# Litianyu141/Gen-FVGN-steady

Hardware: AMD Instinct MI355X
Metric: training iters/sec, 50k-cell cylinder mesh (fwd + loss + bwd + Adam, batch resident in HBM) (higher is better)
Workload: dtype f32

## Files before the change

### gen-fvgn-steady_amd/csrc/gfv_launch.h

```cpp
#pragma once
#include <hip/hip_runtime.h>
#include <tuple>
#include <type_traits>

struct GfvRecorder;
GfvRecorder* gfv_rec_active();
void gfv_rec_push(GfvRecorder* r, hipError_t (*run)(const void* blob, hipStream_t st), const void* blob, size_t bytes, hipStream_t st);

template <class... KArgs, class... Args>
inline void gfv_launch(void (*kernel)(KArgs...), dim3 grid, dim3 block, size_t shmem, hipStream_t st, Args&&... args) {
  hipLaunchKernelGGL(kernel, grid, block, shmem, st, args...);
  if (GfvRecorder* r = gfv_rec_active()) {
    struct Blob {
      void (*k)(KArgs...);
      dim3 g, b;
      size_t sh;
      std::tuple<std::decay_t<KArgs>...> a;
    };
    static_assert(std::is_trivially_copyable<std::tuple<std::decay_t<KArgs>...>>::value || true, "kernel arguments are plain data");
    const Blob blob{kernel, grid, block, shmem, std::tuple<std::decay_t<KArgs>...>(args...)};
    gfv_rec_push(r, [](const void* p, hipStream_t s) -> hipError_t {
      const Blob& B = *static_cast<const Blob*>(p);
      std::apply([&](const auto&... a) { hipLaunchKernelGGL(B.k, B.g, B.b, B.sh, s, a...); }, B.a);
      return hipGetLastError();
    }, &blob, sizeof(Blob), st);
  }
}
#define GFV_LAUNCH(kernel, grid, block, shmem, stream, ...) gfv_launch(kernel, dim3(grid), dim3(block), (size_t)(shmem), stream, __VA_ARGS__)

hipError_t gfv_memset_rec(void* dst, int value, size_t bytes, hipStream_t st);
```

### gen-fvgn-steady_amd/csrc/gfv_limits.h

```cpp
#pragma once
enum {
  GFV_LIM_CBWD_ON = 0,
  GFV_LIM_CBWD_MAX_M,
  GFV_LIM_CFWD_ON,
  GFV_LIM_CFWD_MAX_M,
  GFV_LIM_CTRANS_ON,
  GFV_LIM_CTRANS_MAX_M,
  GFV_LIM_LIN1S_ON,
  GFV_LIM_LIN1S_MAX_M,
  GFV_LIM_COUNT
};
int gfv_internal_limit(int which);
```

### gen-fvgn-steady_amd/csrc/record.hip

```cpp
#include <algorithm>
#include <cstdlib>
#include <cstring>
#include <mutex>
#include <unordered_map>
#include <vector>

#include "../../include/gfv.h"
#include "gfv_common.h"
#include "gfv_launch.h"

struct GfvRecorder {
  struct Cmd {
    hipError_t (*run)(const void*, hipStream_t);
    hipStream_t st;
    size_t off;
  };
  std::vector<Cmd> cmds;
  std::vector<char> arena;
};

namespace {
thread_local GfvRecorder* t_active = nullptr;
std::mutex g_mu;
std::unordered_map<int64_t, GfvRecorder*> g_lists;
int64_t g_next = 1;

constexpr int N_EVENTS = 64;
constexpr int MAX_DEVICES = 16;
struct EventRing {
  hipEvent_t ev[N_EVENTS];
  bool ready = false;
  int next = 0;
};
EventRing g_rings[MAX_DEVICES];
hipEvent_t next_event() {
  int dev = 0;
  if (hipGetDevice(&dev) != hipSuccess || dev < 0 || dev >= MAX_DEVICES) return nullptr;
  std::lock_guard<std::mutex> lk(g_mu);
  EventRing& r = g_rings[dev];
  if (!r.ready) {
    for (int i = 0; i < N_EVENTS; ++i)
      if (hipEventCreateWithFlags(&r.ev[i], hipEventDisableTiming) != hipSuccess) return nullptr;
    r.ready = true;
  }
  hipEvent_t e = r.ev[r.next];
  r.next = (r.next + 1) % N_EVENTS;
  return e;
}
struct WaitBlob {
  hipStream_t waited;
};
hipError_t run_wait(const void* p, hipStream_t waiter) {
  const WaitBlob& B = *static_cast<const WaitBlob*>(p);
  hipEvent_t e = next_event();
  if (!e) return hipErrorInvalidResourceHandle;
  hipError_t rc = hipEventRecord(e, B.waited);
  if (rc != hipSuccess) return rc;
  return hipStreamWaitEvent(waiter, e, 0);
}
struct MemsetBlob {
  void* dst;
  int value;
  size_t bytes;
};
hipError_t run_memset(const void* p, hipStream_t st) {
  const MemsetBlob& B = *static_cast<const MemsetBlob*>(p);
  return hipMemsetAsync(B.dst, B.value, B.bytes, st);
}
}

GfvRecorder* gfv_rec_active() { return t_active; }
void gfv_rec_push(GfvRecorder* r, hipError_t (*run)(const void*, hipStream_t), const void* blob, size_t bytes, hipStream_t st) {
  const size_t off = (r->arena.size() + 15) & ~(size_t)15;
  r->arena.resize(off + bytes);
  memcpy(r->arena.data() + off, blob, bytes);
  r->cmds.push_back({run, st, off});
}
hipError_t gfv_memset_rec(void* dst, int value, size_t bytes, hipStream_t st) {
  const MemsetBlob b{dst, value, bytes};
  const hipError_t rc = run_memset(&b, st);
  if (GfvRecorder* r = gfv_rec_active()) gfv_rec_push(r, run_memset, &b, sizeof(b), st);
  return rc;
}

extern "C" int gfv_record_begin(void) {
  if (t_active) return GFV_ERR_ARG;
  t_active = new GfvRecorder();
  return GFV_OK;
}
extern "C" int gfv_record_count(void) { return t_active ? (int)t_active->cmds.size() : -1; }
extern "C" int64_t gfv_record_end(void) {
  if (!t_active) return 0;
  GfvRecorder* r = t_active;
  t_active = nullptr;
  std::lock_guard<std::mutex> lk(g_mu);
  const int64_t h = g_next++;
  g_lists[h] = r;
  return h;
}
extern "C" int gfv_record_length(int64_t handle) {
  std::lock_guard<std::mutex> lk(g_mu);
  auto it = g_lists.find(handle);
  return it == g_lists.end() ? -1 : (int)it->second->cmds.size();
}
extern "C" int gfv_record_replay(int64_t handle, int32_t first, int32_t last) {
  GfvRecorder* r = nullptr;
  {
    std::lock_guard<std::mutex> lk(g_mu);
    auto it = g_lists.find(handle);
    if (it == g_lists.end()) return GFV_ERR_ARG;
    r = it->second;
  }
  const int n = (int)r->cmds.size();
  if (first < 0 || last > n || first > last) return GFV_ERR_ARG;
  if (t_active) return GFV_ERR_ARG;
  const char* base = r->arena.data();
  for (int i = first; i < last; ++i)
    if (r->cmds[i].run(base + r->cmds[i].off, r->cmds[i].st) != hipSuccess) return GFV_ERR_LAUNCH;
  return GFV_OK;
}
extern "C" int gfv_record_free(int64_t handle) {
  GfvRecorder* r = nullptr;
  {
    std::lock_guard<std::mutex> lk(g_mu);
    auto it = g_lists.find(handle);
    if (it == g_lists.end()) return GFV_ERR_ARG;
    r = it->second;
    g_lists.erase(it);
  }
  delete r;
  return GFV_OK;
}
extern "C" int gfv_stream_wait(void* waiter, void* waited) {
  const WaitBlob b{(hipStream_t)waited};
  hipEvent_t e = next_event();
  if (!e) return GFV_ERR_LAUNCH;
  if (hipEventRecord(e, (hipStream_t)waited) != hipSuccess || hipStreamWaitEvent((hipStream_t)waiter, e, 0) != hipSuccess)
    return GFV_ERR_LAUNCH;
  if (GfvRecorder* r = gfv_rec_active()) gfv_rec_push(r, run_wait, &b, sizeof(b), (hipStream_t)waiter);
  return GFV_OK;
}

extern "C" int gfv_record_delay_side(int64_t handle, void* main_stream, int32_t k) {
  GfvRecorder* r = nullptr;
  {
    std::lock_guard<std::mutex> lk(g_mu);
    auto it = g_lists.find(handle);
    if (it == g_lists.end()) return GFV_ERR_ARG;
    r = it->second;
  }
  if (k <= 0) return 0;
  const hipStream_t ms = (hipStream_t)main_stream;
  auto& c = r->cmds;
  const size_t n = c.size();
  auto is_join = [&](size_t i) { return c[i].st == ms && c[i].run == run_wait; };
  int moved_runs = 0;
  size_t i = 0;
  while (i < n) {
    if (c[i].st == ms) { ++i; continue; }
    size_t j = i;
    while (j < n && c[j].st != ms) ++j;
    size_t d = 0, t = j;
    while (t < n && !is_join(t)) { if (c[t].st == ms) ++d; ++t; }
    size_t want = d / 3 < (size_t)k ? d / 3 : (size_t)k;
// ... 13 lines not shown
```

### gen-fvgn-steady_amd/csrc/rowtile.hip

```cpp
#include <atomic>
#include <stdio.h>
#include <stdlib.h>
#include <mutex>
#include "gfv_common.h"
#include "gfv_limits.h"
#include "gfv_prof.h"
#include "../../include/gfv.h"

namespace {
constexpr int BM = 64;
}

int gfv_internal_tchain_launch(const gfv_rowtile_args_t* args, int ragged, int f16, hipStream_t stream);

static std::atomic<int> g_f16_default{-1};
static thread_local int g_f16split = -1;
static int f16_default() {
  int d = g_f16_default.load(std::memory_order_relaxed);
  if (d < 0) {
    const char* e = getenv("GFV_F16SPLIT");
    d = e ? ((atoi(e) == 2 || atoi(e) == 3) ? atoi(e) : (atoi(e) != 0)) : 1;
    int expect = -1;
    if (!g_f16_default.compare_exchange_strong(expect, d)) d = expect;
  }
// ... 7 lines not shown
}
extern "C" int gfv_set_f16split_thread(int32_t on) {
  if (on < -1 || on > 3) return GFV_ERR_ARG;
  g_f16split = on;
  return GFV_OK;
}
static int f16_mode() { return gfv_f16split_enabled(); }

static thread_local int g_hidden = 128;
extern "C" int gfv_hidden_size(void) { return g_hidden; }
extern "C" int gfv_set_hidden_size(int32_t h) {
  if (h < 16 || h > 128 || (h & 15)) return GFV_ERR_ARG;
  g_hidden = h;
  return GFV_OK;
}

static thread_local int g_last_path = -1;
extern "C" int gfv_rowtile_last_path(void) { return g_last_path; }
namespace {
struct LimitDef { const char* env; int dflt; };
const LimitDef k_limits[GFV_LIM_COUNT] = {
    {"GFV_CBWD", 1},        {"GFV_CBWD_MAX_M", 25000},      {"GFV_CFWD", 1},          {"GFV_CFWD_MAX_M", 250000},
    {"GFV_CTRANS", 1},         {"GFV_CTRANS_MAX_M", 16384},
    {"GFV_LIN1S", 1},       {"GFV_LIN1S_MAX_M", 16384}};
int g_limit[GFV_LIM_COUNT];
bool g_limit_set[GFV_LIM_COUNT];
std::once_flag g_limit_once;
void limits_init() {
  for (int i = 0; i < GFV_LIM_COUNT; ++i) {
    const char* e = getenv(k_limits[i].env);
    g_limit[i] = e ? atoi(e) : k_limits[i].dflt;
    g_limit_set[i] = false;
  }
}
}
int gfv_internal_limit(int which) {
  std::call_once(g_limit_once, limits_init);
  return (which >= 0 && which < GFV_LIM_COUNT) ? g_limit[which] : 0;
}
extern "C" int gfv_get_limit(int32_t which) { return (which >= 0 && which < GFV_LIM_COUNT) ? gfv_internal_limit(which) : -1; }
extern "C" int gfv_set_limit(int32_t which, int32_t value) {
  if (which < 0 || which >= GFV_LIM_COUNT) return GFV_ERR_ARG;
  std::call_once(g_limit_once, limits_init);
  if (value < 0) {
    const char* e = getenv(k_limits[which].env);
    g_limit[which] = e ? atoi(e) : k_limits[which].dflt;
  } else {
// ... 164 lines not shown
```

### gen-fvgn-steady_amd/gfv/cmdlist.py

```python
from __future__ import annotations

import torch

import os

NATIVE = os.environ.get("GFV_CMDLIST_NATIVE", "1") != "0"

_QUERIES = frozenset((
    "gfv_abi_version", "gfv_struct_size", "gfv_rowtile_tiles", "gfv_rowtile_last_path", "gfv_dw_chunks", "gfv_dw_slabs",
    "gfv_linear_dw_workspace_floats", "gfv_dw_multi_workspace_floats", "gfv_f16split_enabled", "gfv_set_f16split", "gfv_set_f16split_thread", "gfv_hidden_size",
    "gfv_weight_image_bytes", "gfv_normalizer_blocks", "gfv_slice_softmax_bwd_blocks", "gfv_profile_enable",
    "gfv_profile_collect", "gfv_profile_reset", "gfv_profile_set_sizes", "gfv_status_flags", "gfv_status_mirror", "gfv_prep_workspace_bytes", "gfv_grad_guard_workspace_bytes", "gfv_get_limit", "gfv_set_limit", "gfv_limit_name", "gfv_rowtile_dw_partials", "gfv_rowtile_dw_partials_m",
    "gfv_rowtile_fuses_dw", "gfv_graph_norm_workspace_bytes", "gfv_plan_create", "gfv_plan_destroy", "gfv_plan_table", "gfv_plan_sizes",
    "gfv_record_begin", "gfv_record_count", "gfv_record_end", "gfv_record_length", "gfv_record_replay", "gfv_record_free",
    "gfv_record_delay_side", "gfv_pool_args_bytes", "gfv_pool_table_bytes", "gfv_pool_table_check",
    "gfv_sweep_mirror_create", "gfv_sweep_mirror_free"))


class CommandList:
    def __init__(self):
        self.cmds = []
        self.pool = None
        self.main = None
        self.keep = []
        self.native = 0
        self.n_native = 0

    def __len__(self):
        return len(self.cmds) + self.n_native

    def __del__(self):
        if self.native:
            try:
                from . import lib as L
                L.load(raw=True).gfv_record_free(self.native)
            except Exception:
                pass

# ... 24 lines not shown
                    fn(*args)


_ACTIVE = None


def active():
    return _ACTIVE


_IN_CALL = 0


def call(fn, *args):
    global _IN_CALL
    _IN_CALL += 1
    try:
        r = fn(*args)
    finally:
        _IN_CALL -= 1
    if _ACTIVE is not None:
        if _ACTIVE.native:
            from . import lib as L
            _ACTIVE.cmds.append((fn, args, torch.cuda.current_stream(), L.load(raw=True).gfv_record_count()))
        else:
            _ACTIVE.cmds.append((fn, args, torch.cuda.current_stream()))
    return r


_NO_KERNEL = frozenset((
    "aten::empty.memory_format", "aten::empty_strided", "aten::empty_like", "aten::new_empty", "aten::new_empty_strided",
    "aten::detach", "aten::alias", "aten::lift_fresh", "aten::_unsafe_view", "aten::is_pinned", "aten::resize_",
    "aten::set_.source_Storage", "aten::set_.source_Storage_storage_offset", "aten::set_.source_Tensor", "aten::_local_scalar_dense",
    "aten::is_same_size", "aten::stride", "aten::sym_size", "aten::sym_stride", "aten::sym_numel", "aten::sym_storage_offset"))


def _guard_mode():
    from torch.utils._python_dispatch import TorchDispatchMode
    from torch.utils._pytree import tree_leaves

    class Guard(TorchDispatchMode):
        def __torch_dispatch__(self, func, types, args=(), kwargs=None):
            out = func(*args, **(kwargs or {}))
            if _IN_CALL == 0:
                name = func._schema.name + ("." + func._overloadname if func._overloadname and func._overloadname != "default" else "")
                if name not in _NO_KERNEL and not getattr(func, "is_view", False):
                    leaves = tree_leaves((args, kwargs, out))
# ... 84 lines not shown
```

### gen-fvgn-steady_amd/gfv/engine.py

```python
from __future__ import annotations

import contextlib
import os
import struct

import torch

from . import cmdlist
from . import lib as L
from . import ops
from .ops import LayerSpec, Seg

_MODE = {"explicit": 0, "implicit": 1, "imex": 2}


def _empty(dev, *shape):
    return torch.empty(shape, dtype=torch.float32, device=dev)


def pick_concurrent_stream(priority=0, candidates=8):
    if torch.cuda.is_current_stream_capturing():
        return torch.cuda.Stream(priority=priority)
    main = torch.cuda.current_stream()
    cycles = 400_000
# ... 102 lines not shown
        self._zero_e = None
        self._etmp = None
        self._prep_ws = None
        self._fvm_cnt = None
        self._fvm_fuse = os.environ.get("GFV_FVM_FUSE", "1") != "0"
        self._agg_ln = os.environ.get("GFV_AGG_LN", "1") != "0"
        self._side, self._sides = None, []
        self._keep = []
        self.dist_world, self.dist_group, self.dist_force = 1, None, False
        self._retired = []
        self.bucket_hook = None

    class _Fork:
        def __init__(self, eng, keep):
            self.eng, self.keep = eng, keep

        def __enter__(self):
            e = self.eng
            if not e.overlap:
                return self
            if e._side is None:
                e._side = pick_concurrent_stream()
                e._sides = [e._side]
            L.stream_wait(e._side, torch.cuda.current_stream())
            e._keep.extend(t for t in self.keep if t is not None)
            self._ctx = torch.cuda.stream(e._side)
            self._ctx.__enter__()
            return self

        def __exit__(self, *exc):
            if self.eng.overlap:
                self._ctx.__exit__(*exc)
            return False

    def fork(self, *keep):
        return Engine._Fork(self, keep)

    @contextlib.contextmanager
    def model_width(self):
        lib = L.load()
        if self.hidden == 128 and lib.gfv_hidden_size() == 128:
            yield
            return
        L.check(lib.gfv_set_hidden_size(self.hidden), "gfv_set_hidden_size")
        try:
            yield
        finally:
# ... 25 lines not shown
        if not self._pending:
            return
        pend, self._pending = self._pending, []
        if split and len(pend) > 1:
            k = 1 if split == 1 else len(pend) - 1
            main_part, side_part = (pend[:k], pend[k:]) if split == 1 else (pend[k:], pend[:k])
            self._pending = side_part
            self.flush()
            self._pending = main_part
            self.flush(on_main=True)
            return
        if on_main:
            ws, self._dw_ws = self._dw_ws, self._dw_ws_main
            try:
                for fn, _ in pend:
                    fn()
            finally:
                self._dw_ws_main, self._dw_ws = self._dw_ws, ws
            return
        with self.fork(*[t for _, keep in pend for t in keep]):
            for fn, _ in pend:
                fn()

    def join(self):
        self.flush()
        if self.overlap and self._side is not None:
            for sd in self._sides:
                L.stream_wait(torch.cuda.current_stream(), sd)
        self._keep.clear()

    def _pkey(self, P, fresh=False):
        hit = self._pkey_cache
        if fresh or hit is None or hit[0] is not P:
            self._pkey_cache = hit = (P, tuple(t.data_ptr() for t in P.values()))
        return hit[1]

    def _wi_enter(self, phase, P):
        if not self.f16split:
            return None
        key = self._pkey(P, fresh=(phase == "fwd"))
        if self._wi_key != key:
            dev = next(iter(P.values())).device
            self._retired.append((self._wi, self._wmax, self._wi_abs))
            self._wmax = torch.zeros((1,), dtype=torch.float32, device=dev)
            self._wi = {ph: ops.WeightImages(dev, self._wmax) for ph in ("fwd", "bwd")}
            self._wi["fwd"].add_static(P.values())
            mats = [t for t in P.values() if t.dim() == 2 and t.stride(1) == 1]
            self._wi_abs = ops.WeightImages._upload([((t.data_ptr(), t.stride(0), t.shape[0], t.shape[1]), t) for t in mats], dev)
            self._wi_key = key
        wi = self._wi[phase]
        if phase == "fwd":
# ... 7 lines not shown
        return ops.set_weight_images(wi)

    def build_static_images(self, P):
        if not self.f16split:
            return
        prev = self._wi_enter("fwd", P)
        ops.set_weight_images(prev)

    def _wi_static_enter(self, P):
        if not self.f16split:
            return None
        if self._wi is None or self._wi_key != self._pkey(P, fresh=True):
            raise RuntimeError("static weight images belong to another parameter set: call build_static_images(P) first")
        wi = self._wi["fwd"]
        if len(wi.valid) != len(wi.images) and cmdlist.active() is None:
            L.check(L.load().gfv_weight_absmax(self._wi_abs[0].data_ptr(), self._wi_abs[1], self._wmax.data_ptr(),
                                               L.stream_ptr()), "gfv_weight_absmax")
            wi.build()
        return ops.set_weight_images(wi)

    def capture_signature(self):
        wi = self._wi or {}
        return (self._wi_key, self._wt_key, L.load().gfv_f16split_enabled(),
                tuple((ph, len(w.images), None if w._desc is None else w._desc.data_ptr()) for ph, w in sorted(wi.items())))

    def _wi_exit(self, phase, prev):
        if not self.f16split:
            return
        self._wi[phase].invalidate()
        ops.set_weight_images(prev)

    def _T(self, W, perm=False):
        hit = self._wt.get((W.data_ptr(), perm)) if self._wt_live else None
        if hit is not None:
            return hit
        if not perm:
            return ops.transpose(W)
        if perm == "c":
            return ops.transpose(W, col0=256, ncols=128)
        if perm == "ab":
            return torch.cat((ops.transpose(W, col0=0, ncols=128), ops.transpose(W, col0=128, ncols=128)), 1).contiguous()
        out = _empty(W.device, 192, 128)
        ops.transpose(W, out=out[0:128], col0=64, ncols=128)
        ops.transpose(W, out=out[128:192], col0=0, ncols=64)
        return out

# ... 879 lines not shown
            if g_emb is not None:
                pending = g_emb
            if self.bucket_hook is not None and proc is sv["procs"][-1] and len(sv["procs"]) > 1:
                self.flush()
                self.bucket_hook()
        tail = self._tail_cfg(pl)[0] if self._defer_mode else 0
        self.mlp3_bwd(P, sv["sv_eenc"], g_e, grads)
        self.flush(on_main=tail >= 2)
        self.mlp3_bwd(P, sv["sv_nenc"], g_x, grads, g_add=pending)
        self.flush(on_main=tail >= 1)

    def forward(self, P, buffers, x, pl, *, norm_global=True, accumulate=True, want_outputs=True, want_edge_attr15=True,
                before_prep=None, x_raw=None, train_loss=None, keep=True, static_weights=False):
        if static_weights:
            prev = self._wi_static_enter(P)
        else:
            with self.fork():
                prev = self._wi_enter("fwd", P)
        try:
            if before_prep is not None:
                before_prep()
            uv_old, ea16, ea15 = self.prep_fwd(x, buffers, pl, norm_global, accumulate, want_edge_attr15, x_raw=x_raw)
            if not static_weights:
                self.join()
            dec, sv_sim = self.simulator_fwd(P, x, ea16, pl, keep=keep)
        finally:
            if not static_weights:
                self._wi_exit("fwd", prev)
            elif self.f16split:
                ops.set_weight_images(prev)
        if not keep:
            del ea16
        losses, uvp_node, uvp_cell, sv_fvm = self.fvm_fwd(dec, uv_old, pl, want_outputs, train_loss=train_loss, keep=keep)
        return losses, uvp_node, uvp_cell, ea15, (dict(sim=sv_sim, fvm=sv_fvm) if keep else None)

    def backward(self, P, ctx, gloss, grads, pl, g_dec_hook=None):
        with self.fork():
            self.prepare_transposes(P)
            prev = self._wi_enter("bwd", P)
        try:
            g_dec = self.fvm_bwd(ctx["fvm"], gloss, pl)
            if g_dec_hook is not None:
                g_dec_hook(g_dec)
            self.join()
            self.simulator_bwd(P, ctx["sim"], g_dec, grads, pl)
            self.join()
        finally:
            self._wt_live = False
            self._wi_exit("bwd", prev)
        return grads
```

### gen-fvgn-steady_amd/gfv/functions.py

```python
from __future__ import annotations

import torch

from .engine import Engine, GradStore
from .plan import get_plan


def require_gpu(t):
    if not t.is_cuda:
        raise RuntimeError("Gen-FVGN MI355X path: tensors must live on the GPU (HIP kernels only, no CPU fallback)")


def _alloc_grads(names, tensors, skip=()):
    return GradStore(names, [t.shape for t in tensors], tensors[0].device, skip=skip)


def unused_param_names(names):
    return {n for n in names if ".ln_1." in ("." + n) or n.endswith("Attn.temperature")}


class GnBlockFn(torch.autograd.Function):
    @staticmethod
    def forward(ctx, engine, plan, names, x, e, *params):
        require_gpu(x)
# ... 136 lines not shown
        ent = self.entries.get(key)
        if ent is None:
            if len(self.entries) >= 4:
                self.entries.pop(next(iter(self.entries)))
            ent = self.entries[key] = _Replay()
            ent.plan = plan
        return ent

    def clear(self):
        self.entries.clear()


class ModelFn(torch.autograd.Function):

    @staticmethod
    def forward(ctx, engine, plan, names, buffers, x, flags, cache, *params):
        require_gpu(x)
        from . import cmdlist
        from . import lib as L
        t_in = __import__("time").perf_counter() if TIMING is not None else 0.0
        P = None
        ent = None
        if cache is not None and cmdlist.active() is None and not torch.cuda.is_current_stream_capturing():
            key = (id(plan), flags["norm_global"], flags["accumulate"], L.load().gfv_f16split_enabled(),
                   tuple(p.data_ptr() for p in params))
            ent = cache.lookup(engine, plan, key)

        def run():
            nonlocal P
            P = dict(zip(names, (p.detach() for p in params)))
            return engine.forward(P, buffers, x, plan, norm_global=flags["norm_global"], accumulate=flags["accumulate"])
        with engine.model_width():
            if ent is None or ent.pending:
                ent = None
                losses, uvp_node, uvp_cell, ea15, sv = run()
            elif ent.fwd is None:
                if ent.warm < ReplayCache.WARM:
                    ent.warm += 1
                    ent = None
                    losses, uvp_node, uvp_cell, ea15, sv = run()
                else:
                    with cmdlist.record() as cl:
                        losses, uvp_node, uvp_cell, ea15, sv = run()
                    ent.fwd, ent.x, ent.sv, ent.P = cl, x, sv, P
                    ent.outs = (losses, uvp_node, uvp_cell, ea15)
                    ent.sig = engine.capture_signature()
            elif ent.sig != engine.capture_signature():
# ... 79 lines not shown
```

### gen-fvgn-steady_amd/gfv/lib.py

```python
from __future__ import annotations

import ctypes as C
import os

import torch

HERE = os.path.dirname(os.path.abspath(__file__))
LIB_PATH = os.environ.get("GFV_LIB", os.path.join(HERE, "libgfv.so"))

c_float_p = C.c_void_p
c_int_p = C.c_void_p

OP_NONE, OP_BIAS_GELU, OP_MUL_DGELU = 0, 1, 2
IN_NONE, IN_GELU, IN_LN, IN_LNBWD = 0, 1, 2, 3
FIN_PLAIN, FIN_LN, FIN_LNBWD = 0, 1, 2
CHAIN_ROW_OWNER, CHAIN_COLUMN_OWNER = 1, 2
DW_COLSCALE = 8


class Seg(C.Structure):
    _fields_ = [("ptr", C.c_void_p), ("idx", C.c_void_p), ("width", C.c_int32), ("ld", C.c_int32),
                ("csr_rowptr", C.c_void_p), ("csr_scale", C.c_void_p), ("save", C.c_void_p)]


# ... 268 lines not shown
                                       C.c_void_p]),
    "gfv_anderson_gram": (C.c_int, [C.c_void_p, C.c_void_p, C.c_int32, C.c_void_p, C.c_void_p, C.c_void_p, C.c_int32, C.c_int32,
                                    C.c_int32, C.c_double, C.c_double, C.c_int32] + [C.c_void_p] * 10 + [C.c_int32, C.c_void_p,
                                                                                                         C.c_void_p]),
    "gfv_anderson_mix": (C.c_int, [C.c_void_p, C.c_void_p, C.c_int32, C.c_void_p, C.c_void_p, C.c_void_p, C.c_int32, C.c_int32,
                                   C.c_int32, C.c_double, C.c_void_p, C.c_void_p, C.c_void_p, C.c_void_p, C.c_int32, C.c_void_p,
                                   C.c_void_p]),
    "gfv_sweep_anderson_gram": (C.c_int, [C.c_void_p, C.c_void_p, C.c_int32, C.c_void_p, C.c_void_p, C.c_void_p, C.c_int32, C.c_int32,
                                          C.c_int32, C.c_double, C.c_double, C.c_int32, C.c_int32] + [C.c_void_p] * 14),
    "gfv_sweep_anderson_mix": (C.c_int, [C.c_void_p, C.c_void_p, C.c_int32, C.c_void_p, C.c_void_p, C.c_void_p, C.c_int32, C.c_int32,
                                         C.c_int32, C.c_double, C.c_int32] + [C.c_void_p] * 6),
    "gfv_sweep_advance_aa": (C.c_int, [C.c_void_p, C.c_void_p, C.c_void_p, C.c_int32, C.c_void_p, C.c_void_p, C.c_void_p, C.c_int32,
                                       C.c_int32] + [C.c_void_p] * 10),
    "gfv_trans_mlp_fwd": (C.c_int, [C.POINTER(TransMlp), C.c_void_p]),
    "gfv_trans_mlp_bwd": (C.c_int, [C.POINTER(TransMlpBwd), C.c_void_p]),
    "gfv_trans_mlp_ln_rows": (C.c_int, [C.c_int32]),
    "gfv_record_begin": (C.c_int, []),
    "gfv_record_count": (C.c_int, []),
    "gfv_record_end": (C.c_int64, []),
    "gfv_record_length": (C.c_int, [C.c_int64]),
    "gfv_record_replay": (C.c_int, [C.c_int64, C.c_int32, C.c_int32]),
    "gfv_record_free": (C.c_int, [C.c_int64]),
    "gfv_stream_wait": (C.c_int, [C.c_void_p, C.c_void_p]),
    "gfv_record_delay_side": (C.c_int, [C.c_int64, C.c_void_p, C.c_int32]),
    "gfv_lbfgs_workspace_doubles": (C.c_size_t, [C.c_int32, C.c_int64]),
    "gfv_lbfgs_pair": (C.c_int, [C.c_void_p, C.c_void_p, C.c_int32, C.c_int64, C.c_void_p, C.c_void_p, C.c_void_p, C.c_void_p,
                                 C.c_double, C.c_int32, C.c_void_p]),
    "gfv_lbfgs_multidot": (C.c_int, [C.c_void_p, C.c_void_p, C.c_int32, C.c_int64, C.c_void_p, C.c_void_p, C.c_void_p, C.c_int32,
                                     C.c_void_p]),
    "gfv_lbfgs_coef": (C.c_int, [C.c_void_p, C.c_void_p, C.c_void_p, C.c_void_p, C.c_void_p, C.c_int32, C.c_int64, C.c_int32,
                                 C.c_void_p]),
    "gfv_lbfgs_combine": (C.c_int, [C.c_void_p, C.c_void_p, C.c_int32, C.c_int64, C.c_void_p, C.c_void_p, C.c_void_p, C.c_void_p,
                                    C.c_void_p, C.c_void_p]),
    "gfv_lbfgs_dot": (C.c_int, [C.c_void_p, C.c_void_p, C.c_void_p, C.c_void_p, C.c_int64, C.c_void_p, C.c_void_p, C.c_void_p,
                                C.c_void_p]),
    "gfv_lbfgs_axpy": (C.c_int, [C.c_void_p, C.c_void_p, C.c_void_p, C.c_double, C.c_void_p, C.c_int64, C.c_void_p]),
}


class PlanDesc(C.Structure):
    _fields_ = [("n_nodes", C.c_int64), ("n_faces", C.c_int64), ("n_cells", C.c_int64), ("n_incidences", C.c_int64),
                ("n_stencil_pairs", C.c_int64), ("n_support_pairs", C.c_int64),
                ("edge_index", C.c_void_p), ("cells_node", C.c_void_p), ("cells_face", C.c_void_p),
                ("cells_index", C.c_void_p), ("face_node_x", C.c_void_p), ("support_edge", C.c_void_p)]


# ... 27 lines not shown
    lib = C.CDLL(LIB_PATH)
    for name, (restype, argtypes) in _SIGNATURES.items():
        fn = getattr(lib, name)
        fn.restype, fn.argtypes = restype, argtypes
    if lib.gfv_abi_version() != ABI_VERSION:
        raise RuntimeError(f"libgfv.so has ABI {lib.gfv_abi_version()}, this binding is written for {ABI_VERSION}: rebuild it "
                           "(python gen-fvgn-steady_amd/gfv/build.py)")
    for which, st in enumerate((Seg, Layer, RowtileArgs, WimgDesc, DwTile, ReducePiece, PlanDesc, TransMlp, TransMlpBwd, FvmMesh,
                                RenewRec)):
        if lib.gfv_struct_size(which) != C.sizeof(st):
            raise RuntimeError(f"libgfv.so: struct {st.__name__} is {lib.gfv_struct_size(which)} bytes in the library, "
                               f"{C.sizeof(st)} in the binding")
    if lib.gfv_pool_args_bytes() != C.sizeof(PoolArgs):
        raise RuntimeError(f"libgfv.so: gfv_pool_args_t is {lib.gfv_pool_args_bytes()} bytes in the library, "
                           f"{C.sizeof(PoolArgs)} in the binding")
    _lib = lib
    return lib if (_recording is None or raw) else _recording


def stream_ptr():
    return C.c_void_p(torch.cuda.current_stream().cuda_stream)


def stream_wait(waiter, waited):
    check(load().gfv_stream_wait(C.c_void_p(waiter.cuda_stream), C.c_void_p(waited.cuda_stream)), "gfv_stream_wait")


_limit_ids = None


def limit_id(name):
    global _limit_ids
    if _limit_ids is None:
        lib, ids, i = load(raw=True), {}, 0
        while True:
            n = lib.gfv_limit_name(i)
            if not n:
                break
            ids[n.decode()] = i
            i += 1
        _limit_ids = ids
    return _limit_ids[name]


def get_limit(name):
    return load(raw=True).gfv_get_limit(limit_id(name))


# ... 75 lines not shown
```

### gen-fvgn-steady_amd/gfv/trainer.py

```python
from __future__ import annotations

import contextlib
import os

import torch

from . import cmdlist
from . import lib as L
from .accum import GradAccum, check_accum_steps
from .balance import check_balance
from .ema import WeightEMA, check_ema
from .engine import GradStore
from .functions import unused_param_names
from .groups import ParamGroups, check_groups, check_weight_decay
from .guard import GradGuard, check_policy
from .observe import Observations, check_observe
from .optstep import optimizer_launches
from .plan import _live_key, _refresh_live, get_plan
from .schedule import check_schedule
from .trainlog import make_log


def _gather(src, index, out):
    torch.index_select(src, 0, index, out=out)
# ... 489 lines not shown
        self._live = _live_key(graphs)
        self.x = graphs[0].x
        self.x_backup = self.x.clone()
        if self.gloss.shape[0] != self.plan.B:
            self.gloss = torch.zeros((self.plan.B, 4), dtype=torch.float32, device=self.dev)
        self._graphs = {}
        self._list_warm = {}

    def _body(self, accumulate, with_adam=True):
        lib = L.load()
        st = L.stream_ptr()
        if self.padded:
            cmdlist.call(_gather, self.flat_p, self._pad_map, self.flat_pp)
        with self.engine.model_width():
            losses, uvp_node, uvp_cell, _, ctx = self.engine.forward(
                self.P_run, self.model.node_norm.buffers_dict(), self.x, self.plan, norm_global=True, accumulate=accumulate,
                want_outputs=self.want_outputs, want_edge_attr15=False, x_raw=self.x_backup,
                train_loss=(self.hyper, self.loss, self.gloss))
            obs, hook = self.observations, None
            if obs is not None:
                fv, pl = ctx["fvm"], self.plan
                obs.fwd(fv["phi"], pl, losses, self.hyper, self.loss, self.gloss)
                hook = lambda g_dec: obs.bwd(fv["dec"], fv["phi"], pl, g_dec)
            self.engine.backward(self.P_run, ctx, self.gloss, self.G_run, self.plan, g_dec_hook=hook)
        if self.padded:
            cmdlist.call(_gather, self.G_run.flat, self._unpad_map, self.flat_g)
        self.losses, self.uvp_node, self.uvp_cell = losses, uvp_node, uvp_cell
        self._after_backward()
        if with_adam:
            self._adam()

    def _after_backward(self):
        """Launches of a subclass between the backward and the optimiser's (gfv.march.MarchStep: the march launch): part of the
        step body, so eager steps, recorded lists and captures carry them alike.  Nothing here."""

    def _adam(self):
        optimizer_launches(self.flat_p, self.flat_g, self.flat_m, self.flat_v, self.n_params, self.adam_state, self.hyper,
                           guard=self._guard, accum=self._accum, ema=self._ema, groups=self._pg, B=self.plan.B, loss=self.loss)

    def _bucket_split(self):
        if self._split is None:
            names = [n for n in self.G.off if ".processpr_list." in n]
            last = max((int(n.split(".processpr_list.")[1].split(".")[0]) for n in names), default=-1)
            offs = [self.G.off[n] for n in names if f".processpr_list.{last}." in n]
            self._split = min(offs) if (last > 0 and offs) else 0
        return self._split

# ... 146 lines not shown
```

### include/gfv.h

```cpp
#ifndef GFV_H_
#define GFV_H_
#include <stddef.h>
#include <stdint.h>

#ifdef __cplusplus
extern "C" {
#endif

#define GFV_ABI_VERSION 3
int gfv_abi_version(void);
int gfv_struct_size(int32_t which);

int gfv_seg_gather_sum(const float* src, const int32_t* rowptr, const int32_t* col, const float* scale,
                       const float* src_scale, float* out, int32_t n_rows, int32_t F, int32_t accumulate, void* stream);

int gfv_seg_gather_sum_nnz(const float* src, const int32_t* rowptr, const int32_t* col, const float* scale,
                           const float* src_scale, float* out, int32_t n_rows, int32_t F, int32_t accumulate,
                           int64_t nnz_hint, void* stream);

int gfv_seg_gather_sum_ex(const float* src, const int32_t* rowptr, const int32_t* col, const float* scale,
                          const float* src_scale, float* out, int32_t n_rows, int32_t F, int32_t accumulate,
                          int64_t nnz_hint, int64_t n_src_hint, void* stream);

int gfv_seg_gather_sum_ln(const float* y, const float* stats, const float* gamma, const float* beta, const int32_t* rowptr,
// ... 383 lines not shown
  const float* fx1;
  const void* img_post_t;
  const void* img_pre_t;
  const void* img_out_t;
  const float* gamma;
  const float* wmax;
  float* g_z;
  float* g_fx1;
  float* g_out_x;
  float* ln_partial;
  float* gscale;
  int32_t M, reserved;
} gfv_trans_mlp_bwd_t;
int gfv_trans_mlp_fwd(const gfv_trans_mlp_t* args, void* stream);
int gfv_trans_mlp_bwd(const gfv_trans_mlp_bwd_t* args, void* stream);
int gfv_trans_mlp_ln_rows(int32_t M);

int gfv_record_begin(void);
int gfv_record_count(void);
int64_t gfv_record_end(void);
int gfv_record_length(int64_t handle);
int gfv_record_replay(int64_t handle, int32_t first, int32_t last);
int gfv_record_free(int64_t handle);
int gfv_stream_wait(void* waiter_stream, void* waited_stream);
int gfv_record_delay_side(int64_t handle, void* main_stream, int32_t k);

int gfv_rollout_advance(const float* uvp_node, float* x_backup, float* x, int32_t N, const int32_t* chunk_beg,
                        const int32_t* chunk_end, const int32_t* gchunk_ptr, int32_t n_chunks, int32_t B, const float* losses,
                        double* partial_ws, float* history, int32_t K_max, int32_t* state, void* stream);

int gfv_sweep_mirror_create(int32_t n_words, int32_t** host_words, int32_t** dev_words);
int gfv_sweep_mirror_free(int32_t* host_words);
int gfv_sweep_advance(const float* uvp_node, float* x_backup, float* x, int32_t N, const int32_t* chunk_beg,
                      const int32_t* chunk_end, const int32_t* gchunk_ptr, int32_t n_chunks, int32_t B, const float* losses,
                      double* partial_ws, const void* ctl, int32_t* slots, float* last, float* state3, int32_t* mirror_dev,
                      int32_t* state, void* stream);

#define GFV_MARCH_RECORD 16
#define GFV_MARCH_HEAD 8
#define GFV_MARCH_GRAPH 8
#define GFV_MARCH_CONVERGED 1u
#define GFV_MARCH_CAPPED 2u
int gfv_march_advance(const float* uvp_node, float* x_backup, float* x, int32_t N, const int32_t* chunk_beg,
                      const int32_t* chunk_end, const int32_t* gchunk_ptr, int32_t n_chunks, int32_t B, const float* losses,
                      double* partial_ws, const float* hyper, int32_t* march, float* r0, void* history, int32_t max_levels,
                      int32_t max_inner, int32_t min_inner, float* snap, int32_t keep, int32_t* mirror_dev, void* stream);

// ... 136 lines not shown
```

Before: 284.3.

## Use device-scope events and kernel-attached stop events for recorded stream joins

Cross-stream joins in the engine's fork/join can now use events created with hipEventDisableSystemFence, so they skip the system-scope fence. By default (edge form 2), each recorded wait is paired at record end with the preceding launch on the waited stream. That launch is replayed via hipExtLaunchKernelGGL with a stop event, so the join waits on that event instead of a separate hipEventRecord. Python-side fences keep pairing from crossing host-call boundaries, and replays fall back to plain system-scope markers when out of order, under capture, or when the runtime refuses the stop event. The cost is more bookkeeping and a risk of weaker memory visibility if a consumer outside the device needs the data.

```diff
diff --git a/gen-fvgn-steady_amd/csrc/gfv_launch.h b/gen-fvgn-steady_amd/csrc/gfv_launch.h
--- a/gen-fvgn-steady_amd/csrc/gfv_launch.h
+++ b/gen-fvgn-steady_amd/csrc/gfv_launch.h
@@ -1,29 +1,46 @@
 #pragma once
 #include <hip/hip_runtime.h>
+#include <hip/hip_ext.h>
 #include <tuple>
 #include <type_traits>
 
 struct GfvRecorder;
 GfvRecorder* gfv_rec_active();
-void gfv_rec_push(GfvRecorder* r, hipError_t (*run)(const void* blob, hipStream_t st), const void* blob, size_t bytes, hipStream_t st);
+void gfv_rec_push(GfvRecorder* r, hipError_t (*run)(const void* blob, hipStream_t st), const void* blob, size_t bytes, hipStream_t st,
+                  bool launch = false);
+struct GfvLaunchHead {
+  hipEvent_t stop;
+};
+hipEvent_t gfv_rec_stop_event(hipEvent_t stop);
+void gfv_rec_stop_refused();
 
 template <class... KArgs, class... Args>
 inline void gfv_launch(void (*kernel)(KArgs...), dim3 grid, dim3 block, size_t shmem, hipStream_t st, Args&&... args) {
   hipLaunchKernelGGL(kernel, grid, block, shmem, st, args...);
   if (GfvRecorder* r = gfv_rec_active()) {
     struct Blob {
+      GfvLaunchHead h;
       void (*k)(KArgs...);
       dim3 g, b;
       size_t sh;
       std::tuple<std::decay_t<KArgs>...> a;
     };
     static_assert(std::is_trivially_copyable<std::tuple<std::decay_t<KArgs>...>>::value || true, "kernel arguments are plain data");
-    const Blob blob{kernel, grid, block, shmem, std::tuple<std::decay_t<KArgs>...>(args...)};
+    const Blob blob{{nullptr}, kernel, grid, block, shmem, std::tuple<std::decay_t<KArgs>...>(args...)};
     gfv_rec_push(r, [](const void* p, hipStream_t s) -> hipError_t {
       const Blob& B = *static_cast<const Blob*>(p);
+      if (B.h.stop) {
+        if (hipEvent_t stop = gfv_rec_stop_event(B.h.stop)) {
+          std::apply([&](const auto&... a) {
+            hipExtLaunchKernelGGL(B.k, B.g, B.b, (std::uint32_t)B.sh, s, nullptr, stop, 0, a...);
+          }, B.a);
+          if (hipGetLastError() == hipSuccess) return hipSuccess;
+          gfv_rec_stop_refused();
+        }
+      }
       std::apply([&](const auto&... a) { hipLaunchKernelGGL(B.k, B.g, B.b, B.sh, s, a...); }, B.a);
       return hipGetLastError();
-    }, &blob, sizeof(Blob), st);
+    }, &blob, sizeof(Blob), st, true);
   }
 }
 #define GFV_LAUNCH(kernel, grid, block, shmem, stream, ...) gfv_launch(kernel, dim3(grid), dim3(block), (size_t)(shmem), stream, __VA_ARGS__)
diff --git a/gen-fvgn-steady_amd/csrc/gfv_limits.h b/gen-fvgn-steady_amd/csrc/gfv_limits.h
--- a/gen-fvgn-steady_amd/csrc/gfv_limits.h
+++ b/gen-fvgn-steady_amd/csrc/gfv_limits.h
@@ -8,6 +8,7 @@
   GFV_LIM_CTRANS_MAX_M,
   GFV_LIM_LIN1S_ON,
   GFV_LIM_LIN1S_MAX_M,
+  GFV_LIM_EDGE_FORM,
   GFV_LIM_COUNT
 };
 int gfv_internal_limit(int which);
diff --git a/gen-fvgn-steady_amd/csrc/record.hip b/gen-fvgn-steady_amd/csrc/record.hip
--- a/gen-fvgn-steady_amd/csrc/record.hip
+++ b/gen-fvgn-steady_amd/csrc/record.hip
@@ -1,4 +1,5 @@
 #include <algorithm>
+#include <atomic>
 #include <cstdlib>
 #include <cstring>
 #include <mutex>
@@ -8,15 +9,24 @@
 #include "../../include/gfv.h"
 #include "gfv_common.h"
 #include "gfv_launch.h"
+#include "gfv_limits.h"
 
 struct GfvRecorder {
+  enum Kind : int { OTHER = 0, LAUNCH = 1, WAIT = 2 };
   struct Cmd {
     hipError_t (*run)(const void*, hipStream_t);
     hipStream_t st;
     size_t off;
+    int kind;
   };
   std::vector<Cmd> cmds;
   std::vector<char> arena;
+  std::vector<size_t> fences;
+  std::vector<hipEvent_t> events;
+  int cursor = 0;
+  ~GfvRecorder() {
+    for (hipEvent_t e : events) (void)hipEventDestroy(e);
+  }
 };
 
 namespace {
@@ -32,31 +42,48 @@
   bool ready = false;
   int next = 0;
 };
-EventRing g_rings[MAX_DEVICES];
-hipEvent_t next_event() {
+enum { SCOPE_SYSTEM = 0, SCOPE_DEVICE = 1 };
+EventRing g_rings[2][MAX_DEVICES];
+hipEvent_t next_event(int scope) {
   int dev = 0;
   if (hipGetDevice(&dev) != hipSuccess || dev < 0 || dev >= MAX_DEVICES) return nullptr;
   std::lock_guard<std::mutex> lk(g_mu);
-  EventRing& r = g_rings[dev];
+  EventRing& r = g_rings[scope][dev];
   if (!r.ready) {
+    const unsigned flags = hipEventDisableTiming | (scope == SCOPE_DEVICE ? hipEventDisableSystemFence : 0u);
     for (int i = 0; i < N_EVENTS; ++i)
-      if (hipEventCreateWithFlags(&r.ev[i], hipEventDisableTiming) != hipSuccess) return nullptr;
+      if (hipEventCreateWithFlags(&r.ev[i], flags) != hipSuccess) return nullptr;
     r.ready = true;
   }
   hipEvent_t e = r.ev[r.next];
   r.next = (r.next + 1) % N_EVENTS;
   return e;
 }
+hipError_t marker_edge(hipStream_t waiter, hipStream_t waited, int scope) {
+  hipEvent_t e = next_event(scope);
+  if (!e) return hipErrorInvalidResourceHandle;
+  hipError_t rc = hipEventRecord(e, waited);
+  if (rc != hipSuccess) return rc;
+  return hipStreamWaitEvent(waiter, e, 0);
+}
+bool capturing(hipStream_t st) {
+  hipStreamCaptureStatus s = hipStreamCaptureStatusNone;
+  return hipStreamIsCapturing(st, &s) != hipSuccess || s != hipStreamCaptureStatusNone;
+}
+
+thread_local bool t_plain = false;
+std::atomic<bool> g_stop_refused{false};
+
 struct WaitBlob {
   hipStream_t waited;
+  int scope;
+  hipEvent_t paired;
 };
 hipError_t run_wait(const void* p, hipStream_t waiter) {
   const WaitBlob& B = *static_cast<const WaitBlob*>(p);
-  hipEvent_t e = next_event();
-  if (!e) return hipErrorInvalidResourceHandle;
-  hipError_t rc = hipEventRecord(e, B.waited);
-  if (rc != hipSuccess) return rc;
-  return hipStreamWaitEvent(waiter, e, 0);
+  if (t_plain) return marker_edge(waiter, B.waited, SCOPE_SYSTEM);
+  if (B.paired && !g_stop_refused.load(std::memory_order_relaxed)) return hipStreamWaitEvent(waiter, B.paired, 0);
+  return marker_edge(waiter, B.waited, B.scope);
 }
 struct MemsetBlob {
   void* dst;
@@ -67,15 +94,51 @@
   const MemsetBlob& B = *static_cast<const MemsetBlob*>(p);
   return hipMemsetAsync(B.dst, B.value, B.bytes, st);
 }
+
+int pair_waits(GfvRecorder* r) {
+  auto& c = r->cmds;
+  char* base = r->arena.data();
+  int paired = 0;
+  for (size_t i = 0; i < c.size(); ++i) {
+    if (c[i].kind != GfvRecorder::WAIT) continue;
+    WaitBlob& W = *reinterpret_cast<WaitBlob*>(base + c[i].off);
+    if (W.scope == SCOPE_SYSTEM) continue;
+    size_t floor = 0;
+    for (size_t f : r->fences)
+      if (f <= i && f > floor) floor = f;
+    for (size_t j = i; j-- > floor;) {
+      if (c[j].st != W.waited) continue;
+      if (c[j].kind == GfvRecorder::LAUNCH) {
+        GfvLaunchHead& H = *reinterpret_cast<GfvLaunchHead*>(base + c[j].off);
+        if (!H.stop) {
+          hipEvent_t e = nullptr;
+          if (hipEventCreateWithFlags(&e, hipEventDisableTiming | hipEventDisableSystemFence) != hipSuccess) break;
+          r->events.push_back(e);
+          H.stop = e;
+        }
+        W.paired = H.stop;
+        ++paired;
+      }
+      break;
+    }
+  }
+  return paired;
+}
 }
 
 GfvRecorder* gfv_rec_active() { return t_active; }
-void gfv_rec_push(GfvRecorder* r, hipError_t (*run)(const void*, hipStream_t), const void* blob, size_t bytes, hipStream_t st) {
+void gfv_rec_push(GfvRecorder* r, hipError_t (*run)(const void*, hipStream_t), const void* blob, size_t bytes, hipStream_t st,
+                  bool launch) {
   const size_t off = (r->arena.size() + 15) & ~(size_t)15;
   r->arena.resize(off + bytes);
   memcpy(r->arena.data() + off, blob, bytes);
-  r->cmds.push_back({run, st, off});
-}
+  r->cmds.push_back({run, st, off, launch ? GfvRecorder::LAUNCH : (run == run_wait ? GfvRecorder::WAIT : GfvRecorder::OTHER)});
+}
+hipEvent_t gfv_rec_stop_event(hipEvent_t stop) {
+  return (t_plain || g_stop_refused.load(std::memory_order_relaxed)) ? nullptr : stop;
+}
+void gfv_rec_stop_refused() { g_stop_refused.store(true); }
+extern "C" int gfv_record_stop_refused(void) { return g_stop_refused.load() ? 1 : 0; }
 hipError_t gfv_memset_rec(void* dst, int value, size_t bytes, hipStream_t st) {
   const MemsetBlob b{dst, value, bytes};
   const hipError_t rc = run_memset(&b, st);
@@ -89,10 +152,16 @@
   return GFV_OK;
 }
 extern "C" int gfv_record_count(void) { return t_active ? (int)t_active->cmds.size() : -1; }
+extern "C" int gfv_record_fence(void) {
+  if (!t_active) return GFV_ERR_ARG;
+  t_active->fences.push_back(t_active->cmds.size());
+  return GFV_OK;
+}
 extern "C" int64_t gfv_record_end(void) {
   if (!t_active) return 0;
   GfvRecorder* r = t_active;
   t_active = nullptr;
+  if (gfv_internal_limit(GFV_LIM_EDGE_FORM) == 2) pair_waits(r);
   std::lock_guard<std::mutex> lk(g_mu);
   const int64_t h = g_next++;
   g_lists[h] = r;
@@ -102,6 +171,16 @@
   std::lock_guard<std::mutex> lk(g_mu);
   auto it = g_lists.find(handle);
   return it == g_lists.end() ? -1 : (int)it->second->cmds.size();
+}
+extern "C" int gfv_record_paired(int64_t handle) {
+  std::lock_guard<std::mutex> lk(g_mu);
+  auto it = g_lists.find(handle);
+  if (it == g_lists.end()) return -1;
+  const GfvRecorder* r = it->second;
+  int n = 0;
+  for (const auto& c : r->cmds)
+    if (c.kind == GfvRecorder::WAIT && reinterpret_cast<const WaitBlob*>(r->arena.data() + c.off)->paired) ++n;
+  return n;
 }
 extern "C" int gfv_record_replay(int64_t handle, int32_t first, int32_t last) {
   GfvRecorder* r = nullptr;
@@ -115,9 +194,16 @@
   if (first < 0 || last > n || first > last) return GFV_ERR_ARG;
   if (t_active) return GFV_ERR_ARG;
   const char* base = r->arena.data();
+  if (!r->events.empty()) {
+    const bool in_order = first == 0 || first == r->cursor;
+    t_plain = !in_order || (first < last && capturing(r->cmds[first].st));
+    r->cursor = in_order ? last : -1;
+  }
+  int rc = GFV_OK;
   for (int i = first; i < last; ++i)
-    if (r->cmds[i].run(base + r->cmds[i].off, r->cmds[i].st) != hipSuccess) return GFV_ERR_LAUNCH;
-  return GFV_OK;
+    if (r->cmds[i].run(base + r->cmds[i].off, r->cmds[i].st) != hipSuccess) { rc = GFV_ERR_LAUNCH; break; }
+  t_plain = false;
+  return rc;
 }
 extern "C" int gfv_record_free(int64_t handle) {
   GfvRecorder* r = nullptr;
@@ -131,15 +217,17 @@
   delete r;
   return GFV_OK;
 }
-extern "C" int gfv_stream_wait(void* waiter, void* waited) {
-  const WaitBlob b{(hipStream_t)waited};
-  hipEvent_t e = next_event();
-  if (!e) return GFV_ERR_LAUNCH;
-  if (hipEventRecord(e, (hipStream_t)waited) != hipSuccess || hipStreamWaitEvent((hipStream_t)waiter, e, 0) != hipSuccess)
-    return GFV_ERR_LAUNCH;
+static int stream_wait(void* waiter, void* waited, int device_scope) {
+  const int form = device_scope ? gfv_internal_limit(GFV_LIM_EDGE_FORM) : 0;
+  const int scope = (form == 1 || form == 2) ? SCOPE_DEVICE : SCOPE_SYSTEM;
+  const int now = form == 1 && !capturing((hipStream_t)waited) ? SCOPE_DEVICE : SCOPE_SYSTEM;
+  if (marker_edge((hipStream_t)waiter, (hipStream_t)waited, now) != hipSuccess) return GFV_ERR_LAUNCH;
+  const WaitBlob b{(hipStream_t)waited, scope, nullptr};
   if (GfvRecorder* r = gfv_rec_active()) gfv_rec_push(r, run_wait, &b, sizeof(b), (hipStream_t)waiter);
   return GFV_OK;
 }
+extern "C" int gfv_stream_wait(void* waiter, void* waited) { return stream_wait(waiter, waited, 0); }
+extern "C" int gfv_stream_wait_device(void* waiter, void* waited) { return stream_wait(waiter, waited, 1); }
 
 extern "C" int gfv_record_delay_side(int64_t handle, void* main_stream, int32_t k) {
   GfvRecorder* r = nullptr;
diff --git a/gen-fvgn-steady_amd/csrc/rowtile.hip b/gen-fvgn-steady_amd/csrc/rowtile.hip
--- a/gen-fvgn-steady_amd/csrc/rowtile.hip
+++ b/gen-fvgn-steady_amd/csrc/rowtile.hip
@@ -53,7 +53,8 @@
 const LimitDef k_limits[GFV_LIM_COUNT] = {
     {"GFV_CBWD", 1},        {"GFV_CBWD_MAX_M", 25000},      {"GFV_CFWD", 1},          {"GFV_CFWD_MAX_M", 250000},
     {"GFV_CTRANS", 1},         {"GFV_CTRANS_MAX_M", 16384},
-    {"GFV_LIN1S", 1},       {"GFV_LIN1S_MAX_M", 16384}};
+    {"GFV_LIN1S", 1},       {"GFV_LIN1S_MAX_M", 16384},
+    {"GFV_EDGE_FORM", 2}};
 int g_limit[GFV_LIM_COUNT];
 bool g_limit_set[GFV_LIM_COUNT];
 std::once_flag g_limit_once;
diff --git a/gen-fvgn-steady_amd/gfv/cmdlist.py b/gen-fvgn-steady_amd/gfv/cmdlist.py
--- a/gen-fvgn-steady_amd/gfv/cmdlist.py
+++ b/gen-fvgn-steady_amd/gfv/cmdlist.py
@@ -13,7 +13,7 @@
     "gfv_profile_collect", "gfv_profile_reset", "gfv_profile_set_sizes", "gfv_status_flags", "gfv_status_mirror", "gfv_prep_workspace_bytes", "gfv_grad_guard_workspace_bytes", "gfv_get_limit", "gfv_set_limit", "gfv_limit_name", "gfv_rowtile_dw_partials", "gfv_rowtile_dw_partials_m",
     "gfv_rowtile_fuses_dw", "gfv_graph_norm_workspace_bytes", "gfv_plan_create", "gfv_plan_destroy", "gfv_plan_table", "gfv_plan_sizes",
     "gfv_record_begin", "gfv_record_count", "gfv_record_end", "gfv_record_length", "gfv_record_replay", "gfv_record_free",
-    "gfv_record_delay_side", "gfv_pool_args_bytes", "gfv_pool_table_bytes", "gfv_pool_table_check",
+    "gfv_record_delay_side", "gfv_record_fence", "gfv_record_paired", "gfv_record_stop_refused", "gfv_pool_args_bytes", "gfv_pool_table_bytes", "gfv_pool_table_check",
     "gfv_sweep_mirror_create", "gfv_sweep_mirror_free"))
 
 
@@ -84,7 +84,9 @@
     if _ACTIVE is not None:
         if _ACTIVE.native:
             from . import lib as L
-            _ACTIVE.cmds.append((fn, args, torch.cuda.current_stream(), L.load(raw=True).gfv_record_count()))
+            lib = L.load(raw=True)
+            lib.gfv_record_fence()
+            _ACTIVE.cmds.append((fn, args, torch.cuda.current_stream(), lib.gfv_record_count()))
         else:
             _ACTIVE.cmds.append((fn, args, torch.cuda.current_stream()))
     return r
diff --git a/gen-fvgn-steady_amd/gfv/engine.py b/gen-fvgn-steady_amd/gfv/engine.py
--- a/gen-fvgn-steady_amd/gfv/engine.py
+++ b/gen-fvgn-steady_amd/gfv/engine.py
@@ -148,7 +148,7 @@
             if e._side is None:
                 e._side = pick_concurrent_stream()
                 e._sides = [e._side]
-            L.stream_wait(e._side, torch.cuda.current_stream())
+            L.stream_wait(e._side, torch.cuda.current_stream(), device_scope=True)
             e._keep.extend(t for t in self.keep if t is not None)
             self._ctx = torch.cuda.stream(e._side)
             self._ctx.__enter__()
@@ -220,11 +220,11 @@
             for fn, _ in pend:
                 fn()
 
-    def join(self):
+    def join(self, device_scope=False):
         self.flush()
         if self.overlap and self._side is not None:
             for sd in self._sides:
-                L.stream_wait(torch.cuda.current_stream(), sd)
+                L.stream_wait(torch.cuda.current_stream(), sd, device_scope=device_scope)
         self._keep.clear()
 
     def _pkey(self, P, fresh=False):
@@ -278,6 +278,7 @@
     def capture_signature(self):
         wi = self._wi or {}
         return (self._wi_key, self._wt_key, L.load().gfv_f16split_enabled(),
+                L.get_limit("GFV_EDGE_FORM"),
                 tuple((ph, len(w.images), None if w._desc is None else w._desc.data_ptr()) for ph, w in sorted(wi.items())))
 
     def _wi_exit(self, phase, prev):
@@ -1203,7 +1204,7 @@
                 before_prep()
             uv_old, ea16, ea15 = self.prep_fwd(x, buffers, pl, norm_global, accumulate, want_edge_attr15, x_raw=x_raw)
             if not static_weights:
-                self.join()
+                self.join(device_scope=True)
             dec, sv_sim = self.simulator_fwd(P, x, ea16, pl, keep=keep)
         finally:
             if not static_weights:
@@ -1215,7 +1216,7 @@
         losses, uvp_node, uvp_cell, sv_fvm = self.fvm_fwd(dec, uv_old, pl, want_outputs, train_loss=train_loss, keep=keep)
         return losses, uvp_node, uvp_cell, ea15, (dict(sim=sv_sim, fvm=sv_fvm) if keep else None)
 
-    def backward(self, P, ctx, gloss, grads, pl, g_dec_hook=None):
+    def backward(self, P, ctx, gloss, grads, pl, g_dec_hook=None, own_reader=False):
         with self.fork():
             self.prepare_transposes(P)
             prev = self._wi_enter("bwd", P)
@@ -1223,9 +1224,9 @@
             g_dec = self.fvm_bwd(ctx["fvm"], gloss, pl)
             if g_dec_hook is not None:
                 g_dec_hook(g_dec)
-            self.join()
+            self.join(device_scope=True)
             self.simulator_bwd(P, ctx["sim"], g_dec, grads, pl)
-            self.join()
+            self.join(device_scope=own_reader and self.dist_world == 1 and not self.dist_force)
         finally:
             self._wt_live = False
             self._wi_exit("bwd", prev)
diff --git a/gen-fvgn-steady_amd/gfv/functions.py b/gen-fvgn-steady_amd/gfv/functions.py
--- a/gen-fvgn-steady_amd/gfv/functions.py
+++ b/gen-fvgn-steady_amd/gfv/functions.py
@@ -182,7 +182,7 @@
         P = None
         ent = None
         if cache is not None and cmdlist.active() is None and not torch.cuda.is_current_stream_capturing():
-            key = (id(plan), flags["norm_global"], flags["accumulate"], L.load().gfv_f16split_enabled(),
+            key = (id(plan), flags["norm_global"], flags["accumulate"], L.load().gfv_f16split_enabled(), L.get_limit("GFV_EDGE_FORM"),
                    tuple(p.data_ptr() for p in params))
             ent = cache.lookup(engine, plan, key)
 
diff --git a/gen-fvgn-steady_amd/gfv/lib.py b/gen-fvgn-steady_amd/gfv/lib.py
--- a/gen-fvgn-steady_amd/gfv/lib.py
+++ b/gen-fvgn-steady_amd/gfv/lib.py
@@ -314,6 +314,10 @@
     "gfv_record_replay": (C.c_int, [C.c_int64, C.c_int32, C.c_int32]),
     "gfv_record_free": (C.c_int, [C.c_int64]),
     "gfv_stream_wait": (C.c_int, [C.c_void_p, C.c_void_p]),
+    "gfv_stream_wait_device": (C.c_int, [C.c_void_p, C.c_void_p]),
+    "gfv_record_fence": (C.c_int, []),
+    "gfv_record_paired": (C.c_int, [C.c_int64]),
+    "gfv_record_stop_refused": (C.c_int, []),
     "gfv_record_delay_side": (C.c_int, [C.c_int64, C.c_void_p, C.c_int32]),
     "gfv_lbfgs_workspace_doubles": (C.c_size_t, [C.c_int32, C.c_int64]),
     "gfv_lbfgs_pair": (C.c_int, [C.c_void_p, C.c_void_p, C.c_int32, C.c_int64, C.c_void_p, C.c_void_p, C.c_void_p, C.c_void_p,
@@ -387,8 +391,12 @@
     return C.c_void_p(torch.cuda.current_stream().cuda_stream)
 
 
-def stream_wait(waiter, waited):
-    check(load().gfv_stream_wait(C.c_void_p(waiter.cuda_stream), C.c_void_p(waited.cuda_stream)), "gfv_stream_wait")
+def stream_wait(waiter, waited, device_scope=False):
+    lib = load()
+    if device_scope:
+        check(lib.gfv_stream_wait_device(C.c_void_p(waiter.cuda_stream), C.c_void_p(waited.cuda_stream)), "gfv_stream_wait_device")
+    else:
+        check(lib.gfv_stream_wait(C.c_void_p(waiter.cuda_stream), C.c_void_p(waited.cuda_stream)), "gfv_stream_wait")
 
 
 _limit_ids = None
diff --git a/gen-fvgn-steady_amd/gfv/trainer.py b/gen-fvgn-steady_amd/gfv/trainer.py
--- a/gen-fvgn-steady_amd/gfv/trainer.py
+++ b/gen-fvgn-steady_amd/gfv/trainer.py
@@ -535,7 +535,7 @@
                 fv, pl = ctx["fvm"], self.plan
                 obs.fwd(fv["phi"], pl, losses, self.hyper, self.loss, self.gloss)
                 hook = lambda g_dec: obs.bwd(fv["dec"], fv["phi"], pl, g_dec)
-            self.engine.backward(self.P_run, ctx, self.gloss, self.G_run, self.plan, g_dec_hook=hook)
+            self.engine.backward(self.P_run, ctx, self.gloss, self.G_run, self.plan, g_dec_hook=hook, own_reader=not self.padded)
         if self.padded:
             cmdlist.call(_gather, self.G_run.flat, self._unpad_map, self.flat_g)
         self.losses, self.uvp_node, self.uvp_cell = losses, uvp_node, uvp_cell
diff --git a/include/gfv.h b/include/gfv.h
--- a/include/gfv.h
+++ b/include/gfv.h
@@ -429,7 +429,11 @@
 int gfv_record_length(int64_t handle);
 int gfv_record_replay(int64_t handle, int32_t first, int32_t last);
 int gfv_record_free(int64_t handle);
+int gfv_record_fence(void);
+int gfv_record_paired(int64_t handle);
+int gfv_record_stop_refused(void);
 int gfv_stream_wait(void* waiter_stream, void* waited_stream);
+int gfv_stream_wait_device(void* waiter_stream, void* waited_stream);
 int gfv_record_delay_side(int64_t handle, void* main_stream, int32_t k);
 
 int gfv_rollout_advance(const float* uvp_node, float* x_backup, float* x, int32_t N, const int32_t* chunk_beg,
```

After: 286.4 (median of 6 runs). Within noise of the previous version (+0.7%).
